# yhz0/SQLP

Hardware: AMD Instinct MI355X
Metric: stage-2 subproblems/sec + cut-gen HBM GB/s on STORM (higher is better)
Workload: dtype f64

## Files before the change

sqlp_amd/csrc/lp_batch.hip:

```cpp
#include <hip/hip_runtime.h>
#include <algorithm>
#include <cmath>
#include <cstdio>
#include <cstdlib>
#include <vector>
#include "twosd_internal.h"
#include "twosd_ctx.h"

using namespace twosd;

int twosd::run_lp(twosd_ctx *c, const double *x, const double *d_dv, int N, const LpRun &o) {
    const bool want_pi = o.want_pi, want_y = o.want_y;
    const bool list = o.d_list != nullptr;
    const int NL = list ? o.nlist : N;
    int rc;
    if (o.want_ray && !list) return fail(TWOSD_E_ARG, "LP rays: list mode only");
    if ((rc = prepare_x(c, x))) return rc;
    if (list &&c->bp.bases.size() > 1 && (size_t)N > c->d_pool_pick.cap) return fail(TWOSD_E_STATE, "LP list mode: no recorded pool picks");
    const int m = c->L.m, n = c->L.n, MP = c->MP, R = c->R;
    if (N > c->out_cap) {
        size_t cap = std::max<size_t>(N, 1024);
        if ((rc = c->d_obj.alloc(cap)) || (rc = c->d_status.alloc(cap)) || (rc = c->d_iters.alloc(cap)) ||
            (rc = c->d_ops.alloc(cap)) || (rc = c->d_etan.alloc(cap)))
            return rc;
// ... 17 lines not shown
        int bpc = hyper_max_blocks_per_cu(R, CH, kmax, c->k);
        if (const char *e = getenv("TWOSD_BPC")) bpc = std::min(bpc, std::max(1, atoi(e)));
        if (bpc < 1)
            return fail(TWOSD_E_UNSUPPORTED, "LP kernel: LDS slice too large (m2 = %d, n2 = %d; LP: %d rows, %d columns; k = %d)",
                        c->m2_user, c->n2_user, m, n, c->k);
        const int nblocks = std::max(1, std::min((NL + kWavesPerBlock - 1) / kWavesPerBlock, bpc * c->num_cus));
        const size_t slots = (size_t)nblocks * kWavesPerBlock;
        if (slots > c->earena_slots || ecap != c->earena_cap) {
            if ((rc = c->d_eidx.alloc(slots * ecap)) || (rc = c->d_evals.alloc(slots * ecap))) return rc;
            c->earena_slots = slots;
            c->earena_cap = ecap;
        }
        HIPCHK(hipMemsetAsync(c->d_queue, 0, sizeof(int) * kMaxQueueGroups * kQueueStride, c->stream));
        HyperParams H{};
        H.m = m; H.n = n; H.k = c->k; H.N = NL; H.kmax = kmax; H.ecap = ecap;
        H.kcap = o.kcap > 0 ? std::min(o.kcap, kmax) : kmax;
        H.retry = o.kcap > 0 ? 0 : 1;
        H.colptr = c->d_colptr; H.rowidx = c->d_rowidx; H.val = c->d_val; H.q = c->d_q; H.btype = c->d_btype;
        H.wcp = c->d_wcp; H.wcc = c->d_wcc; H.wcv = c->d_wcv;
        const PoolArrays pa = pool_arrays(c);
        H.bcp = pa.bcp; H.bci = pa.bci; H.bcv = pa.bcv;
        H.brptr = pa.brptr; H.brcol = pa.brcol; H.brval = pa.brval;
        H.kslot = pa.kslot; H.kix = pa.kix; H.kv = pa.kv; H.kcoef = c->d_kcoef;
        H.xbase = c->d_xbase; H.d0 = pa.d0; H.hb0 = pa.hb0;
        H.basic0 = pa.basic0; H.fixedmask = c->d_fixedmask; H.ubmask = c->d_ubmask;
        H.dv = d_dv; H.eidx = c->d_eidx; H.evals = c->d_evals; H.queue = c->d_queue;
        H.qgroups = std::max(1, std::min(16, nblocks));
        if (const char *e = getenv("TWOSD_QGROUPS")) H.qgroups = std::max(1, std::min({kMaxQueueGroups, nblocks, atoi(e)}));
        H.obj = c->d_obj; H.pi = want_pi ? c->d_pi : nullptr; H.y = want_y ? c->d_y : nullptr;
        H.vkey = o.want_key ? c->d_vkey : nullptr;
        H.key_zero = 1e-12;
        if (const char *e = getenv("TWOSD_KEY_ZERO")) H.key_zero = atof(e);
        H.bkey = o.want_bkey ? c->d_bkey : nullptr;
        if (o.want_etas) {
            const size_t need = list ? (size_t)NL : (size_t)N;
            if (need * 4096 > (size_t)INT32_MAX)
                return fail(TWOSD_E_UNSUPPORTED, "eta files of %zu solves exceed the 2^31-entry arena (at most %d)", need,
                            INT32_MAX / 4096);
            const size_t cap_need = std::max(std::max<size_t>(need, 256) * 4096, c->eo_min_cap);
            if (need > c->eo_rows || c->eo_kmax != kmax || c->eo_cap < cap_need) {
                const size_t rows = std::max<size_t>(need, 256);
                if ((rc = c->d_eo_pb.alloc(rows)) || (rc = c->d_eo_K.alloc(rows)) || (rc = c->d_eo_off.alloc(rows)) ||
                    (rc = c->d_eo_etap.alloc(rows * kmax)) || (rc = c->d_eo_etaoff.alloc(rows * (kmax + 1))) ||
                    (rc = c->d_eo_eidx.alloc(cap_need)) || (rc = c->d_eo_evals.alloc(cap_need)))
                    return rc;
                if (!c->d_eo_used && (rc = c->d_eo_used.alloc(1))) return rc;
                c->eo_rows = rows;
                c->eo_cap = cap_need;
                c->eo_kmax = kmax;
            }
            HIPCHK(hipMemsetAsync(c->d_eo_used, 0, sizeof(unsigned long long), c->stream));
            H.eo_pb = c->d_eo_pb; H.eo_K = c->d_eo_K; H.eo_off = c->d_eo_off; H.eo_etap = c->d_eo_etap;
            H.eo_etaoff = c->d_eo_etaoff; H.eo_eidx = c->d_eo_eidx; H.eo_evals = c->d_eo_evals; H.eo_used = c->d_eo_used;
            H.eo_cap = (long long)std::min<size_t>(c->eo_cap, INT32_MAX);
        }
        if (o.want_head) {
            const size_t need = list ? (size_t)NL : (size_t)N;
            if ((rc = c->d_head_out.fit(need * m))) return rc;
            H.head_out = c->d_head_out;
        }
        if (o.want_ray) {
            FrayState &Fs = c->fray;
            if ((rc = Fs.ray.fit((size_t)NL * m)) || (rc = Fs.ray_row.fit((size_t)NL)) || (rc = Fs.ray_key.fit((size_t)NL))) return rc;
            HIPCHK(hipMemsetAsync(Fs.ray_row, 0xff, sizeof(int) * NL, c->stream));
            HIPCHK(hipMemsetAsync(Fs.ray_key, 0, sizeof(unsigned long long) * NL, c->stream));
            H.ray = Fs.ray; H.ray_row = Fs.ray_row; H.ray_key = Fs.ray_key;
// ... 291 lines not shown
    if (row_ops) *row_ops = c->last.ops_sum;
    if (row_width) *row_width = 1;
    return TWOSD_OK;
}

__global__ void gather_rows_kernel(int U, int m, const int *__restrict__ list, const double *__restrict__ pi, double *__restrict__ out) {
    const size_t tot = (size_t)U * m;
    for (size_t i = (size_t)blockIdx.x * blockDim.x + threadIdx.x; i < tot; i += (size_t)gridDim.x * blockDim.x) {
        const int u = (int)(i / m), r = (int)(i % m);
        out[i] = pi[(size_t)list[u] * m + r];
    }
}

__global__ void list_status_kernel(int U, const int *__restrict__ list, const int *__restrict__ st,
                                   unsigned long long *bad) {
    for (int i = blockIdx.x * blockDim.x + threadIdx.x; i < U; i += gridDim.x * blockDim.x)
        if (st[list[i]] != TWOSD_LP_OPTIMAL) atomicAdd(bad, 1ull);
}

extern "C" int twosd_solve_push(twosd_ctx *c, int epi, const double *x, int first, int count, double *obj, int *status,
                                int *new_size) {
    if (!c || !c->has_template) return fail(TWOSD_E_STATE, "solve_push: no template");
    if (!c->bp.has_basis) return fail(TWOSD_E_STATE, "solve_push: no warm-start basis");
    if (epi < 0 || epi >= (int)c->epis.size()) return fail(TWOSD_E_ARG, "solve_push: epigraph %d does not exist", epi);
    const EpiDevice &E = c->epis[epi];
    if (first < 0 || count < 0 || first + count > E.count) return fail(TWOSD_E_ARG, "solve_push: range outside the epigraph");
    if (c->n1 > 0 && !x) return fail(TWOSD_E_ARG, "solve_push: x is NULL");
    if (count == 0) { if (new_size) *new_size = c->dvs.size; return TWOSD_OK; }
    HIPCHK(hipSetDevice(c->device));
    const double *d_dv = E.d_dv + (size_t)first * c->k;
    const bool all = getenv("TWOSD_PUSH_ALL") && atoi(getenv("TWOSD_PUSH_ALL")) != 0;
    const int pmode = getenv("TWOSD_PUSH_MODE") ? atoi(getenv("TWOSD_PUSH_MODE")) : 0;
    const bool full = !all && (pmode == 2 || (pmode == 0 && c->push_rep_frac > 0.25));
    c->last_push_full = full ? 1 : 0;
    LpRun o;
    o.want_pi = all || full;
    o.want_key = !all;
    int rc = run_lp(c, x, d_dv, count, o);
    if (rc) return rc;
    rc = copy_lp_outputs(c, count, obj, nullptr, nullptr, status, E.d_w + first);
    if (rc) return rc;
    float ms = 0, ms_key = 0;
    const auto timed_push = [c](int n, const double *d_rows, float *ms_out) -> int {
        HIPCHK(hipEventRecord(c->ev[EV_PUSH_BEGIN], c->stream));
        if (int r = dvs_push_device(c, n, d_rows, nullptr)) return r;
        HIPCHK(hipEventRecord(c->ev[EV_PUSH_END], c->stream));
        HIPCHK(hipEventSynchronize(c->ev[EV_PUSH_END]));
        hipEventElapsedTime(ms_out, c->ev[EV_PUSH_BEGIN], c->ev[EV_PUSH_END]);
        return TWOSD_OK;
    };
    if (all) {
        if ((rc = timed_push(count, c->d_pi, &ms))) return rc;
        c->last_push_reps = count;
    } else {
        HIPCHK(hipEventRecord(c->ev[EV_MARK_1], c->stream));
        const int *d_list = nullptr;
        int U = 0;
        if ((rc = vkey_first_occurrences(c, count, c->d_vkey, c->d_status, &d_list, &U))) return rc;
        HIPCHK(hipEventRecord(c->ev[EV_MARK_2], c->stream));
        HIPCHK(hipEventSynchronize(c->ev[EV_MARK_2]));
        hipEventElapsedTime(&ms_key, c->ev[EV_MARK_1], c->ev[EV_MARK_2]);
        c->last_push_reps = U;
        c->push_rep_frac = (double)U / count;
        if (U > 0 && full) {
            const int m = c->L.m;
            if ((rc = c->d_pi_rep.fit((size_t)U * m))) return rc;
            hipLaunchKernelGGL(gather_rows_kernel, dim3((unsigned)std::min<size_t>(4096, ((size_t)U * m + 255) / 256)), dim3(256), 0,
                               c->stream, U, m, d_list, c->d_pi, c->d_pi_rep);
            HIPCHK(hipGetLastError());
            if ((rc = timed_push(U, c->d_pi_rep, &ms))) return rc;
        } else if (U > 0) {
            double resolve_us = 0.0;
            LpRun r;
            r.want_pi = true;
            r.d_list = d_list;
            r.nlist = U;
            r.lp_us_out = &resolve_us;
            if ((rc = run_lp(c, x, d_dv, count, r))) return rc;
            HIPCHK(hipMemsetAsync(c->d_lpstats, 0, sizeof(unsigned long long), c->stream));
            hipLaunchKernelGGL(list_status_kernel, dim3((unsigned)std::min(256, (U + 255) / 256)), dim3(256), 0, c->stream, U,
                               d_list, c->d_status, c->d_lpstats);
            HIPCHK(hipGetLastError());
            unsigned long long bad = 0;
            HIPCHK(hipMemcpyAsync(&bad, c->d_lpstats, sizeof(bad), hipMemcpyDeviceToHost, c->stream));
            HIPCHK(hipStreamSynchronize(c->stream));
            if (bad) return fail(TWOSD_E_LP, "solve_push: %llu of %d re-solved representatives not optimal; nothing pushed", bad, U);
            c->last.lp_us += resolve_us;
            if ((rc = timed_push(U, c->d_pi, &ms))) return rc;
        }
    }
    c->t_us[T_DEDUP] = 1e3 * (ms + ms_key);
    if (new_size) *new_size = c->dvs.size;
    return TWOSD_OK;
}

extern "C" int twosd_last_push_mode(twosd_ctx *c, int *full) {
    if (!c || !full) return fail(TWOSD_E_ARG, "last_push_mode: NULL");
// ... 10 lines not shown
```

sqlp_amd/csrc/lp_hyper.hip:

```cpp
#include <hip/hip_runtime.h>
#include <math.h>
#include <type_traits>
#include "twosd_internal.h"
#include "wave_ops.h"

namespace twosd {

#define HTOL_P 1e-9
#define HTOL_D 1e-9
#define HTOL_PIV 1e-9
#define HPI_ZERO 1e-12


#ifdef TWOSD_STAMPS
#define STAMP_DECL unsigned long long st_acc[10] = {0, 0, 0, 0, 0, 0, 0, 0, 0, 0}; \
    unsigned long long st_last = __builtin_amdgcn_s_memtime();
#define STAMP(i)                                                      \
    {                                                                 \
        const unsigned long long t_ = __builtin_amdgcn_s_memtime();   \
        st_acc[i] += t_ - st_last;                                    \
        st_last = t_;                                                 \
    }
#define STAMP_FLUSH                                                                         \
    if (lane == 0 && P.stamps)                                                              \
// ... 116 lines not shown

__device__ __forceinline__ const __attribute__((address_space(4))) HyperParams *h_args() {
    uint64_t a = (uint64_t)__builtin_amdgcn_kernarg_segment_ptr();
    asm volatile("" : "+s"(a));
    return (const __attribute__((address_space(4))) HyperParams *)a;
}
#define CP (*h_args())

static __host__ __device__ inline int hyper_union_doubles(int R, int C) {
    return 128 * R > 64 * C ? 128 * R : 64 * C;
}
static __host__ __device__ inline size_t hyper_slice_bytes(int R, int C, int kmax, int k) {
    const int kmaxp = (kmax + 3) & ~3;
    return 8 * (size_t)hyper_union_doubles(R, C) + 8 * (size_t)((k + 1) & ~1) + 8 * 64 + 4 * 64 + 4 * 64 + 2 * kmaxp +
           4 * (kmaxp + 4);
}
size_t hyper_lds_bytes(int R, int C, int kmax, int k) { return (size_t)kWavesPerBlock * hyper_slice_bytes(R, C, kmax, k); }

#ifndef TWOSD_ETA_G
#define TWOSD_ETA_G 2
#endif
constexpr int EG = TWOSD_ETA_G;
#ifndef TWOSD_REC_UNROLL
#define TWOSD_REC_UNROLL 1
#endif
#ifndef TWOSD_XB_U
#define TWOSD_XB_U 1
#endif
constexpr int XU = TWOSD_XB_U;
#ifndef TWOSD_HYPER_WPE
#define TWOSD_HYPER_WPE(R) ((R) >= 9 ? 2 : 3)
#endif

template <int R, int C, bool FULL, bool RAY = false>
__global__ void __launch_bounds__(256, TWOSD_HYPER_WPE(R)) lp_hyper_kernel(HyperParams P) {
    extern __shared__ double lds_raw[];
    using Mask = typename std::conditional<(C > 32), uint64_t, uint32_t>::type;
    const int lane = threadIdx.x & 63;
    const int wid = threadIdx.x >> 6;
    constexpr int MP = 64 * R;
    constexpr int UD = 128 * R > 64 * C ? 128 * R : 64 * C;
    const int kmaxp = (P.kmax + 3) & ~3;
    const int ncol = P.n + P.m;
    char *slice = reinterpret_cast<char *>(lds_raw) + (size_t)wid * hyper_slice_bytes(R, C, P.kmax, P.k);
    double *ut = reinterpret_cast<double *>(slice);
    double *rho = ut + MP;
    double *alpha = ut;
    double *dvl = ut + UD;
    double *lstv = dvl + ((P.k + 1) & ~1);
    int *lsti = reinterpret_cast<int *>(lstv + 64);
    int *smark = lsti + 64;
    unsigned short *etap = reinterpret_cast<unsigned short *>(smark + 64);
    int *etaoff = reinterpret_cast<int *>(etap + kmaxp);

    const int m = P.m, n = P.n;
    const int slot_id = blockIdx.x * kWavesPerBlock + wid;
    int *eidx = P.eidx + (size_t)slot_id * P.ecap;
    double *evals = P.evals + (size_t)slot_id * P.ecap;
    const uint64_t fixedm = CP.fixedmask[lane];
    const uint64_t ubm = CP.ubmask[lane];

    for (int j = lane; j < UD; j += 64) ut[j] = 0.0;
    smark[lane] = 0;
    h_wave_sync();
    STAMP_DECL

    const int G = CP.qgroups;
    const int g0 = blockIdx.x % G;
// ... 539 lines not shown
                {
                    const int nh = q * 4 + (int)P.btype[q];
                    const bool rme = lane == (r & 63);
                    H_SLOT_SWITCH(__builtin_amdgcn_readfirstlane(r >> 6), R, {
                        int v = rme ? nh : hb[SL];
                        asm volatile("" : "+v"(v));
                        hb[SL] = v;
                    })
                }
            }
            ++it;
            h_wave_sync();
            STAMP(8)
        }
        if (status == TWOSD_LP_OPTIMAL || pb == 0 || !CP.retry) break;
        if (lane == 0 && CP.retries) atomicAdd(CP.retries, 1ull);
        pb = 0;
        }
        double dvn0 = 0.0, dvn1 = 0.0, kcn0 = 0.0, kcn1 = 0.0;
        int ksn = 0, t_claim = 0;
        if (q_nx >= 0) {
            const auto *A = h_args();
            t_claim = claim_issue();
            if (lane <= R) ksn = A->kslot[pb_nx * (R + 1) + lane];
            if (dv_pf) {
                const double *dvs = A->dv + (size_t)s_nx * P.k;
                if (lane < P.k) { dvn0 = dvs[lane]; kcn0 = A->kcoef[lane]; }
                if (lane + 64 < P.k) { dvn1 = dvs[lane + 64]; kcn1 = A->kcoef[lane + 64]; }
            }
        }

        double objv = NAN;
        unsigned long long keyv = 0;
        if (status == TWOSD_LP_OPTIMAL) {
            const double *qc = CP.q;
            double qv[R];
#pragma unroll
            for (int t = 0; t < R; ++t) {
                const int j = hb[t] >> 2;
                qv[t] = qc[(hb[t] >= 0 && j < n) ? j : 0];
            }
            double ob = 0.0;
#pragma unroll
            for (int t = 0; t < R; ++t) {
                const int j = hb[t] >> 2;
                ob = (hb[t] >= 0 && j < n) ? fma(qv[t], xB[t], ob) : ob;
            }
            objv = wsum(ob);
        }
        q_n2 = -1;
        if (q_nx >= 0) {
            q_n2 = claim_resolve(t_claim);
            if (lane <= R) lsti[lane] = ksn;
            if (dv_pf) {
                if (lane < P.k) dvl[lane] = kcn0 * dvn0;
                if (lane + 64 < P.k) dvl[lane + 64] = kcn1 * dvn1;
            }
        }
        h_wave_sync();
        if (status == TWOSD_LP_OPTIMAL) {
            if (CP.vkey) {
                uint64_t ub = ubm;
                int lane = threadIdx.x & 63;
                asm volatile("" : "+v"(ub), "+v"(lane));
                auto dk = [&](int c) -> double {
                    const int j = 64 * c + lane;
                    const bool slack = (j >= n) & (j < ncol) & (((bmask >> c) & 1) == 0);
                    return slack ? h_flip(d[c], ((ub >> c) & 1) << 63) : 0.0;
                };
                double pm = 0.0;
#pragma unroll
                for (int c = 0; c < C; ++c) pm = fmax(pm, fabs(dk(c)));
                pm = wmax(pm);
                const double zt = CP.key_zero * (1.0 + pm);
                unsigned long long h = 0;
#pragma unroll
                for (int c = 0; c < C; ++c) {
                    const int j = 64 * c + lane;
                    if (j >= n && j < ncol) {
                        const double dc = dk(c);
                        const double v = fabs(dc) <= zt ? 0.0 : dc;
                        const unsigned long long b = ((unsigned long long)__double_as_longlong(v) + (1ull << 28)) >> 29;
                        h += mix64(((unsigned long long)(j - n) << 35) | b);
                    }
                }
#pragma unroll
                for (int o = 32; o > 0; o >>= 1) h += __shfl_xor(h, o);
                keyv = h;
            }
        }
        if constexpr (FULL) {
        bool rayrec = false;
        if constexpr (RAY) rayrec = status == TWOSD_LP_INFEASIBLE && CP.ray != nullptr;
        if ((status == TWOSD_LP_OPTIMAL && (P.pi || P.y)) || rayrec) {
            if (rayrec) {
                if (lane == (ray_r & 63)) ut[ray_r] = 1.0;
            } else {
                const double *qc = CP.q;
#pragma unroll
                for (int t = 0; t < R; ++t) {
                    const int j = hb[t] >> 2;
                    const bool bq = hb[t] >= 0 && j < n;
                    const double qj = qc[bq ? j : 0];
                    ut[64 * t + lane] = bq ? qj : 0.0;
                }
            }
            h_wave_sync();
            for (int tt = K - 1; tt >= 0; --tt) {
                const int off = etaoff[tt], nnz = etaoff[tt + 1] - off;
                double acc = 0.0;
                for (int e = lane; e < nnz; e += 64) acc = fma(ut[eidx[off + e]], evals[off + e], acc);
                acc = wsum(acc);
                nops += nnz;
                if (lane == 0) ut[etap[tt]] = acc;
                h_wave_sync();
            }
            double pv[R];
            double pmax = 0.0;
#pragma unroll
            for (int t = 0; t < R; ++t) {
                const int cc = 64 * t + lane;
                const int e0 = cc < m ? bcp[cc] : 0, e1 = cc < m ? bcp[cc + 1] : 0;
                double a = 0.0;
#pragma unroll TWOSD_REC_UNROLL
                for (int e = e0; e < e1; ++e) a = fma(ut[P.bci[e]], P.bcv[e], a);
                pv[t] = a;
                pmax = fmax(pmax, fabs(a));
            }
            nops += P.bnnz[pb];
            pmax = wmax(pmax);
            const double zt = HPI_ZERO * (1.0 + pmax);
#pragma unroll
            for (int t = 0; t < R; ++t)
                if (fabs(pv[t]) <= zt) pv[t] = 0.0;
            h_wave_sync();
#pragma unroll
            for (int t = 0; t < R; ++t) ut[64 * t + lane] = 0.0;
            if constexpr (RAY) {
                if (rayrec) {
                    const auto *A = h_args();
                    const size_t ro = (size_t)(P.pi_by_pos ? qpos : s);
                    double *po = A->ray + ro * m;
                    const uint64_t sm = ray_up ? 0ull : (1ull << 63);
                    unsigned long long h = 0;
#pragma unroll
                    for (int t = 0; t < R; ++t)
                        if (64 * t + lane < m) {
                            po[64 * t + lane] = pv[t] == 0.0 ? 0.0 : h_flip(pv[t], sm);
                            h += mix64((unsigned long long)(hb[t] >> 2));
                        }
#pragma unroll
                    for (int o = 32; o > 0; o >>= 1) h += __shfl_xor(h, o);
                    const int leaving = h_get_row_i<R>(hb, ray_r) >> 2;
                    if (lane == 0) {
                        if (A->ray_row) A->ray_row[ro] = ray_r;
                        if (A->ray_key) A->ray_key[ro] = mix64(h ^ mix64(((unsigned long long)leaving << 1) | (ray_up ? 1ull : 0ull)));
                    }
                }
            }
            if (!rayrec && P.pi) {
                double *po = P.pi + (size_t)(P.pi_by_pos ? qpos : s) * m;
#pragma unroll
                for (int t = 0; t < R; ++t)
                    if (64 * t + lane < m) po[64 * t + lane] = pv[t];
            }
            if (!rayrec && P.y) {
                double *yo = P.y + (size_t)s * n;
                for (int j = lane; j < n; j += 64) yo[j] = 0.0;
                __builtin_amdgcn_s_waitcnt(0);
                __builtin_amdgcn_wave_barrier();
// ... 332 lines not shown
__global__ void __launch_bounds__(256) queue_records_kernel(int N, const int *__restrict__ order, const int *__restrict__ pick,
                                                           int2 *__restrict__ qrec) {
    const int q = blockIdx.x * blockDim.x + threadIdx.x;
    if (q >= N) return;
    const int s = order ? order[q] : q;
    qrec[q] = make_int2(s, pick ? pick[s] : 0);
}
hipError_t launch_queue_records(const int *order, const int *pick, int2 *qrec, int N, hipStream_t s) {
    if (N <= 0) return hipSuccess;
    hipLaunchKernelGGL(queue_records_kernel, dim3((N + 255) / 256), dim3(256), 0, s, N, order, pick, qrec);
    return hipGetLastError();
}

static const int kHR[] = {1, 2, 4, 9, 16};
static const int kHC[] = {2, 4, 8, 14, 16, 28, 32, 64};

int hyper_rows_per_lane(int m) {
    for (int R : kHR)
        if (m <= 64 * R) return R;
    return -1;
}
int hyper_cols_per_lane(int ncols) {
    for (int C : kHC)
        if (ncols <= 64 * C) return C;
    return -1;
}

template <int R, int C>
static hipError_t hl(const HyperParams &p, int nb, size_t lds, hipStream_t s) {
    if (p.ray)
        hipLaunchKernelGGL((lp_hyper_kernel<R, C, true, true>), dim3(nb), dim3(256), lds, s, p);
    else if (p.pi || p.y || p.head_out || p.bkey || p.eo_K)
        hipLaunchKernelGGL((lp_hyper_kernel<R, C, true>), dim3(nb), dim3(256), lds, s, p);
    else
        hipLaunchKernelGGL((lp_hyper_kernel<R, C, false>), dim3(nb), dim3(256), lds, s, p);
    return hipGetLastError();
}
template <int R, int C>
static int ho(size_t lds) {
    int nb = 0, nb2 = 0;
    if (hipOccupancyMaxActiveBlocksPerMultiprocessor(&nb, lp_hyper_kernel<R, C, true>, 256, lds) != hipSuccess) return 1;
    if (hipOccupancyMaxActiveBlocksPerMultiprocessor(&nb2, lp_hyper_kernel<R, C, false>, 256, lds) != hipSuccess) return 1;
    nb = std::min(nb, nb2);
    return nb > 0 ? nb : 1;
}

#ifdef HYP_DEV_STORM_ONLY
#define HYPER_C_SWITCH(R, FN, ...)                  \
    switch (C) {                                    \
        case 28: if (R == 9) return FN<9, 28>(__VA_ARGS__); \
    }
#else
#define HYPER_C_SWITCH(R, FN, ...)                  \
    switch (C) {                                    \
        case 2: return FN<R, 2>(__VA_ARGS__);       \
        case 4: return FN<R, 4>(__VA_ARGS__);       \
        case 8: return FN<R, 8>(__VA_ARGS__);       \
        case 14: return FN<R, 14>(__VA_ARGS__);     \
        case 16: return FN<R, 16>(__VA_ARGS__);     \
        case 28: return FN<R, 28>(__VA_ARGS__);     \
        case 32: return FN<R, 32>(__VA_ARGS__);     \
        case 64: return FN<R, 64>(__VA_ARGS__);     \
    }
#endif

hipError_t launch_hyper(int R, int C, const HyperParams &p, int nblocks, size_t lds, hipStream_t s) {
    switch (R) {
        case 1: HYPER_C_SWITCH(1, hl, p, nblocks, lds, s); break;
        case 2: HYPER_C_SWITCH(2, hl, p, nblocks, lds, s); break;
        case 4: HYPER_C_SWITCH(4, hl, p, nblocks, lds, s); break;
        case 9: HYPER_C_SWITCH(9, hl, p, nblocks, lds, s); break;
        case 16: HYPER_C_SWITCH(16, hl, p, nblocks, lds, s); break;
    }
    return hipErrorInvalidValue;
}

// ... 15 lines not shown
```

sqlp_amd/csrc/twosd_ctx.h:

```cpp
#pragma once
#include <hip/hip_runtime.h>
#include <stdint.h>
#include <algorithm>
#include <memory>
#include <thread>
#include <vector>
#include "devbuf.h"
#include "twosd_internal.h"
#include "basis_pool.h"

#define HIPCHK(expr)                                                                                      \
    do {                                                                                                  \
        hipError_t _e = (expr);                                                                           \
        if (_e != hipSuccess) return twosd::fail(TWOSD_E_DEVICE, "%s: %s", #expr, hipGetErrorString(_e)); \
    } while (0)

namespace twosd {

enum StageSlot : int {
    STG_POOL_RCOL = 0, STG_POOL_CROW, STG_POOL_RVAL, STG_POOL_CVAL, STG_POOL_D0,
    STG_ELEM_KE, STG_ELEM_KIX, STG_ELEM_KRAW, STG_ELEM_KV,
    STG_PG_TOT,
    STG_FREE_10,
    STG_PG_NZ,
// ... 236 lines not shown
    twosd::DevBuf<char> d_rt_pack;
    twosd::DevBuf<int> d_gs_heads, d_gs_cnt, d_gs_tot, d_gs_valid, d_gs_irow;
    twosd::DevBuf<long long> d_gs_ioff;
    twosd::DevBuf<double> d_gs_ival;
    twosd::DevBuf<char> d_gs_seg;
    int last_push_reps = 0;
    double push_rep_frac = 0.0;
    int last_push_full = 0;
    twosd::DevBuf<double> d_pi_rep;
    twosd::FrayState fray;
    twosd::RiskState risk;
};

struct twosd_ctx : TemplateState {
    int device = 0;
    hipStream_t stream = nullptr;
    hipEvent_t ev[twosd::EV_COUNT] = {};
    int num_cus = 256;
    int kmax_override = 0;
    int train_kcap = 0;
    twosd::PinnedBuf stage[twosd::STG_COUNT];
    ~twosd_ctx() {
        for (hipEvent_t e : ev)
            if (e) hipEventDestroy(e);
        if (stream) hipStreamDestroy(stream);
    }
};

namespace twosd {
int fail(int code, const char *fmt, ...);
int prepare_x(twosd_ctx *c, const double *x);
struct LpRun {
    bool want_pi = false, want_y = false, want_key = false;
    bool want_bkey = false;
    bool want_etas = false;
    bool want_head = false;
    const int *d_list = nullptr;
    int nlist = 0;
    int kcap = 0;
    double *lp_us_out = nullptr;
    bool want_ray = false;
};
int run_lp(twosd_ctx *c, const double *x, const double *d_dv, int N, const LpRun &o = LpRun());
#pragma GCC visibility push(hidden)
double template_value(const twosd_ctx *c, int e);
void rhs_at(const twosd_ctx *c, const double *x, const double *dv, std::vector<double> &b);
SampleParams sample_params(const twosd_ctx *c, int n, uint64_t seed, uint64_t first_index, double *out);
int draw_scenarios(twosd_ctx *c, int n, uint64_t seed, uint64_t first_index, double *out, int mode, int G);
int upload_lintr(twosd_ctx *c, const LintrTables &T);
int select_pool(twosd_ctx *c, const double *d_dv, int N, int *d_pick, int npool_override);
int copy_lp_outputs(twosd_ctx *c, int N, double *obj, double *pi, double *y, int *status, const double *d_w);
int prepare_elements(twosd_ctx *c);
int reserve_selection(twosd_ctx *c, int P, int records);
void reset_candidates(twosd_ctx *c);
int training_box(twosd_ctx *c, const EpiDevice &E, int epi, int first, int count, std::vector<double> &lo,
                 std::vector<double> &hi, BoxCache *cache);
#pragma GCC visibility pop
template <typename F>
void parallel_for(int n, F f, int serial_below = 64) {
    const int nth = (int)std::max(1u, std::min(16u, std::thread::hardware_concurrency()));
    if (n < serial_below || nth == 1) {
        for (int i = 0; i < n; ++i) f(i);
        return;
    }
    std::vector<std::thread> th;
    for (int t = 0; t < nth; ++t)
        th.emplace_back([&, t]() {
            for (int i = t; i < n; i += nth) f(i);
        });
    for (auto &t : th) t.join();
}
int vkey_first_occurrences(twosd_ctx *c, int N, const unsigned long long *d_vkey, const int *d_status, const int **d_list,
                           int *U, const int **d_counts = nullptr);
int dvs_init(twosd_ctx *c);
int dvs_push_device(twosd_ctx *c, int count, const double *d_pis, int *d_out_index);
void cut_invalidate_pk(twosd_ctx *c);
void cut_truncate_pk(twosd_ctx *c, int size);
int cut_last_usable(twosd_ctx *c, int epi, const char *who, const char *verb);
const int *cut_last_arg(twosd_ctx *c);
int cut_pk_current(twosd_ctx *c, const double **PK, int *k4);
const double *cut_last_val(twosd_ctx *c);
struct RiskResult { double var, cvar; unsigned long long tail_q, total_q; long long n_bad, n_ok; };
int risk_select(twosd_ctx *c, long long n, const double *d_val, const double *d_w, const int *d_st, double scale, bool has_add,
                double add, double level, const char *who, RiskResult *out);
int risk_form_y(twosd_ctx *c, long long n, double *d_obj, const int *d_st, double var, double denom);
int sampling_plan(const twosd_sampling *plan, const char *who, int *mode, int *G);
int whole_groups(const char *who, const char *what, unsigned long long value, int G);
}
```

sqlp_amd/csrc/twosd_internal.h:

```cpp
#pragma once
#include <hip/hip_runtime.h>
#include <stdint.h>
#include <string>
#include <vector>
#include "twosd_hip.h"
#include "devbuf.h"
#include "dist_tables.h"
#include "lintr_tables.h"
#include "pool_pack.h"

namespace twosd {

constexpr int kWave = 64;
constexpr int kWavesPerBlock = 4;
constexpr int kMaxColsPerLane = 64;

enum : int { BT_Y = 0, BT_G = 1, BT_L = 2, BT_E = 3 };


constexpr int kQueueStride = 32;
constexpr int kMaxQueueGroups = 64;
struct HyperParams {
    int m, n, k, N, kmax, ecap;
    int kcap;
    int retry;
    const int *colptr, *rowidx; const double *val;
    const double *q; const int8_t *btype;
    const int *wcp, *wcc; const double *wcv;
    const int *bcp, *bci; const double *bcv;
    const int *brptr, *brcol; const double *brval;
    const int *kslot, *kix; const double *kv;
    const double *kcoef;
    const double *xbase;
    const double *d0;
    const int *hb0;
    const uint64_t *basic0, *fixedmask, *ubmask;
    const double *dv;
    int *eidx; double *evals;
    int *queue;
    int qgroups;
    double *obj;
    int *status, *iters;
    long long *ops;
    int *etan;
    int *pool_pick;
    unsigned long long *vkey;
    double *pi, *y;
    unsigned long long *retries;
    unsigned long long *stamps;
    int npool;
    const int *bnnz;
    int *head_out;
    const int2 *qrec;
    double key_zero;
    int pi_by_pos;
    unsigned long long *bkey;
    int *eo_pb, *eo_K, *eo_off, *eo_etap, *eo_etaoff;
    int *eo_eidx; double *eo_evals;
    unsigned long long *eo_used; long long eo_cap;
    double *ray;
    int *ray_row;
    unsigned long long *ray_key;
};

struct PgArgs {
    int m, n, MP, CH, R9, k, kmax, npool_old;
    const int *colptr, *rowidx; const double *val, *q; const int8_t *btype; const int *pos_row;
    const int *bcp0, *bci0; const double *bcv0;
    const int *eo_pb, *eo_K, *eo_off, *eo_etap, *eo_etaoff, *eo_eidx; const double *eo_evals;
    const int *head0, *heads;
    const int *src_row;
    const int *gheads;
    int a0;
    double *amax;
    int *nzc, *keptc;
    int *nztot;
    const long long *inter_off;
    int *inter_row; double *inter_val;
    int *rowcnt, *erowcnt;
    int *tot;
    int *valid;
    long long sc_cap;
    int *sc_row, *sc_off; double *sc_val;
};
struct PgTable {
    int nsrc;
    int *cnt, *tot, *valid;
    long long *ioff;
    int *irow;
    double *ival;
    int *gheads;
    static size_t plane_size(int nsrc, int m) { return (size_t)nsrc * m; }
    static size_t cnt_size(int nsrc, int m) { return 4 * plane_size(nsrc, m); }
    static size_t tot_size(int nsrc) { return (size_t)5 * nsrc; }
    int *plane(int f, int m) const { return cnt + f * plane_size(nsrc, m); }
// ... 123 lines not shown
```

sqlp_amd/csrc/vkey.hip:

```cpp
#include <hip/hip_runtime.h>
#include <hipcub/hipcub.hpp>
#include <algorithm>
#include "twosd_ctx.h"

namespace twosd {

__device__ __forceinline__ unsigned long long vk_norm(unsigned long long k) { return k ? k : 1ull; }
__device__ __forceinline__ unsigned vk_slot(unsigned long long k, unsigned mask) {
    return (unsigned)((k * 0x9E3779B97F4A7C15ull) >> 32) & mask;
}

__global__ void vkey_clear_kernel(unsigned long long *keys, int *first, int *cnt, unsigned cap) {
    for (unsigned i = blockIdx.x * blockDim.x + threadIdx.x; i < cap; i += gridDim.x * blockDim.x) {
        keys[i] = 0ull;
        first[i] = 0x7fffffff;
        cnt[i] = 0;
    }
}

constexpr int kVkItems = 2048;
constexpr int kVkLds = 2 * kVkItems;
__global__ void __launch_bounds__(256) vkey_insert_kernel(int N, const unsigned long long *__restrict__ vkey,
                                                          const int *__restrict__ status, unsigned long long *keys,
                                                          int *first, int *cnt, unsigned mask) {
    __shared__ unsigned long long lk[kVkLds];
    __shared__ int lf[kVkLds], lc[kVkLds];
    for (int i = threadIdx.x; i < kVkLds; i += blockDim.x) {
        lk[i] = 0ull;
        lf[i] = 0x7fffffff;
        lc[i] = 0;
    }
    __syncthreads();
    const int s0 = blockIdx.x * kVkItems, s1 = min(N, s0 + kVkItems);
    for (int s = s0 + threadIdx.x; s < s1; s += blockDim.x) {
        if (status[s] != TWOSD_LP_OPTIMAL) continue;
        const unsigned long long k = vk_norm(vkey[s]);
        unsigned i = vk_slot(k, kVkLds - 1);
        for (;;) {
            const unsigned long long old = atomicCAS(&lk[i], 0ull, k);
            if (old == 0ull || old == k) {
                atomicMin(&lf[i], s);
                atomicAdd(&lc[i], 1);
                break;
// ... 23 lines not shown
                                  int *out) {
    for (int a = blockIdx.x * blockDim.x + threadIdx.x; a < U; a += gridDim.x * blockDim.x) {
        const unsigned long long k = vk_norm(vkey[list[a]]);
        unsigned i = vk_slot(k, mask);
        while (keys[i] != k) i = (i + 1) & mask;
        out[a] = cnt[i];
    }
}

__global__ void vkey_flag_kernel(int N, const unsigned long long *__restrict__ vkey, const int *__restrict__ status,
                                 const unsigned long long *__restrict__ keys, const int *__restrict__ first,
                                 unsigned mask, char *flag) {
    for (int s = blockIdx.x * blockDim.x + threadIdx.x; s < N; s += gridDim.x * blockDim.x) {
        char f = 0;
        if (status[s] == TWOSD_LP_OPTIMAL) {
            const unsigned long long k = vk_norm(vkey[s]);
            unsigned i = vk_slot(k, mask);
            while (keys[i] != k) i = (i + 1) & mask;
            f = first[i] == s;
        }
        flag[s] = f;
    }
}

template <typename T>
using WsBuf = DevBuf<T, 8>;
struct VkeyWs {
    WsBuf<unsigned long long> keys;
    WsBuf<int> first, cnt;
    unsigned cap = 0;
    WsBuf<char> flag;
    WsBuf<int> list, counts, nsel;
    WsBuf<char> tmp;
};

static VkeyWs *vws(twosd_ctx *c) {
    if (!c->vkey_ws) c->vkey_ws.reset(new VkeyWs());
    return c->vkey_ws.get();
}

void vkey_free(VkeyWs *w) { delete w; }

int vkey_first_occurrences(twosd_ctx *c, int N, const unsigned long long *d_vkey, const int *d_status, const int **d_list,
                           int *U, const int **d_counts) {
    VkeyWs *w = vws(c);
    unsigned cap = 1024;
    while (cap < 2u * (unsigned)N) cap <<= 1;
    int rc;
    if (cap > w->cap) {
        w->cap = 0;
        if ((rc = w->keys.alloc(cap)) || (rc = w->first.alloc(cap)) || (rc = w->cnt.alloc(cap))) return rc;
        w->cap = cap;
    }
    if ((rc = w->flag.fit((size_t)N)) || (rc = w->list.fit((size_t)N)) || (rc = w->counts.fit((size_t)N))) return rc;
    if (!w->nsel && (rc = w->nsel.alloc(1))) return rc;
    size_t need = 0;
    HIPCHK(hipcub::DeviceSelect::Flagged(nullptr, need, hipcub::CountingInputIterator<int>(0), w->flag.p, w->list.p, w->nsel.p, N,
                                         c->stream));
    if ((rc = w->tmp.fit(need))) return rc;
    const unsigned mask = w->cap - 1;
    const int nb = std::max(1, std::min(4096, (N + 255) / 256));
    hipLaunchKernelGGL(vkey_clear_kernel, dim3(std::min(4096u, (w->cap + 255) / 256)), dim3(256), 0, c->stream, w->keys, w->first,
                       w->cnt, w->cap);
    hipLaunchKernelGGL(vkey_insert_kernel, dim3(std::max(1, (N + kVkItems - 1) / kVkItems)), dim3(256), 0, c->stream, N, d_vkey, d_status,
                       w->keys, w->first, w->cnt, mask);
    hipLaunchKernelGGL(vkey_flag_kernel, dim3(nb), dim3(256), 0, c->stream, N, d_vkey, d_status, w->keys, w->first, mask,
                       w->flag);
    HIPCHK(hipGetLastError());
    HIPCHK(hipcub::DeviceSelect::Flagged(w->tmp.p, need, hipcub::CountingInputIterator<int>(0), w->flag.p, w->list.p, w->nsel.p, N,
                                         c->stream));
    HIPCHK(hipMemcpyAsync(U, w->nsel, sizeof(int), hipMemcpyDeviceToHost, c->stream));
    HIPCHK(hipStreamSynchronize(c->stream));
    *d_list = w->list;
    if (d_counts) {
        if (*U > 0) {
            hipLaunchKernelGGL(vkey_count_kernel, dim3(std::max(1, std::min(4096, (*U + 255) / 256))), dim3(256), 0, c->stream, *U,
                               w->list, d_vkey, w->keys, w->cnt, mask, w->counts);
            HIPCHK(hipGetLastError());
        }
        *d_counts = w->counts;
    }
    return TWOSD_OK;
}

}
```

Before: 18.26 million.

## Dedupe dual keys inside the LP kernel and recover duals only for representatives

Adds a REP variant of the lean hyper-sparse LP kernel. Each solve computes its dual key, claims a slot in a global hash table with atomics, and only the lowest-index owner of each key recovers and writes its dual vector, so push no longer needs a separate full dual-recovery pass or host-side dedupe kernels in the common mode. A small winner/gather pass then selects the final representatives, with a fallback to the old vkey path if the table overflows or counts disagree. The cost is extra atomics and global traffic inside the kernel, some wasted recoveries when a lower-index owner arrives later, and a third kernel variant that may lower the occupancy chosen for all variants.

```diff
diff --git a/sqlp_amd/csrc/lp_batch.hip b/sqlp_amd/csrc/lp_batch.hip
--- a/sqlp_amd/csrc/lp_batch.hip
+++ b/sqlp_amd/csrc/lp_batch.hip
@@ -73,6 +73,7 @@
         H.key_zero = 1e-12;
         if (const char *e = getenv("TWOSD_KEY_ZERO")) H.key_zero = atof(e);
         H.bkey = o.want_bkey ? c->d_bkey : nullptr;
+        if (o.want_rep && o.want_key && !list && !want_pi && !want_y && (rc = rep_prepare(c, N, H))) return rc;
         if (o.want_etas) {
             const size_t need = list ? (size_t)NL : (size_t)N;
             if (need * 4096 > (size_t)INT32_MAX)
@@ -430,10 +431,12 @@
     const bool all = getenv("TWOSD_PUSH_ALL") && atoi(getenv("TWOSD_PUSH_ALL")) != 0;
     const int pmode = getenv("TWOSD_PUSH_MODE") ? atoi(getenv("TWOSD_PUSH_MODE")) : 0;
     const bool full = !all && (pmode == 2 || (pmode == 0 && c->push_rep_frac > 0.25));
+    const bool inpass = !all && !full && (pmode == 3 || pmode == 0);
     c->last_push_full = full ? 1 : 0;
     LpRun o;
     o.want_pi = all || full;
     o.want_key = !all;
+    o.want_rep = inpass;
     int rc = run_lp(c, x, d_dv, count, o);
     if (rc) return rc;
     rc = copy_lp_outputs(c, count, obj, nullptr, nullptr, status, E.d_w + first);
@@ -454,13 +457,20 @@
         HIPCHK(hipEventRecord(c->ev[EV_MARK_1], c->stream));
         const int *d_list = nullptr;
         int U = 0;
-        if ((rc = vkey_first_occurrences(c, count, c->d_vkey, c->d_status, &d_list, &U))) return rc;
+        bool got = false;
+        if (inpass && (rc = rep_winners(c, count, c->d_vkey, &U, &got))) return rc;
+        if (!got) {
+            if ((rc = vkey_first_occurrences(c, count, c->d_vkey, c->d_status, &d_list, &U))) return rc;
+            if (inpass) rep_note_reps(c, U);
+        }
         HIPCHK(hipEventRecord(c->ev[EV_MARK_2], c->stream));
         HIPCHK(hipEventSynchronize(c->ev[EV_MARK_2]));
         hipEventElapsedTime(&ms_key, c->ev[EV_MARK_1], c->ev[EV_MARK_2]);
         c->last_push_reps = U;
         c->push_rep_frac = (double)U / count;
-        if (U > 0 && full) {
+        if (U > 0 && got) {
+            if ((rc = timed_push(U, c->d_pi_rep, &ms))) return rc;
+        } else if (U > 0 && full) {
             const int m = c->L.m;
             if ((rc = c->d_pi_rep.fit((size_t)U * m))) return rc;
             hipLaunchKernelGGL(gather_rows_kernel, dim3((unsigned)std::min<size_t>(4096, ((size_t)U * m + 255) / 256)), dim3(256), 0,
diff --git a/sqlp_amd/csrc/lp_hyper.hip b/sqlp_amd/csrc/lp_hyper.hip
--- a/sqlp_amd/csrc/lp_hyper.hip
+++ b/sqlp_amd/csrc/lp_hyper.hip
@@ -172,8 +172,97 @@
 #define TWOSD_HYPER_WPE(R) ((R) >= 9 ? 2 : 3)
 #endif
 
-template <int R, int C, bool FULL, bool RAY = false>
+template <int R>
+__device__ __forceinline__ void h_recover(double (&pv)[R], const HyperParams &P, bool rayrec, int ray_r, const int (&hb)[R], int K,
+                                          int pb, double *ut, const int *etaoff, const unsigned short *etap, const int *eidx,
+                                          const double *evals, const int *bcp, unsigned &nops, int lane) {
+    const int m = P.m, n = P.n;
+    if (rayrec) {
+        if (lane == (ray_r & 63)) ut[ray_r] = 1.0;
+    } else {
+        const double *qc = CP.q;
+#pragma unroll
+        for (int t = 0; t < R; ++t) {
+            const int j = hb[t] >> 2;
+            const bool bq = hb[t] >= 0 && j < n;
+            const double qj = qc[bq ? j : 0];
+            ut[64 * t + lane] = bq ? qj : 0.0;
+        }
+    }
+    h_wave_sync();
+    for (int tt = K - 1; tt >= 0; --tt) {
+        const int off = etaoff[tt], nnz = etaoff[tt + 1] - off;
+        double acc = 0.0;
+        for (int e = lane; e < nnz; e += 64) acc = fma(ut[eidx[off + e]], evals[off + e], acc);
+        acc = wsum(acc);
+        nops += nnz;
+        if (lane == 0) ut[etap[tt]] = acc;
+        h_wave_sync();
+    }
+    double pmax = 0.0;
+#pragma unroll
+    for (int t = 0; t < R; ++t) {
+        const int cc = 64 * t + lane;
+        const int e0 = cc < m ? bcp[cc] : 0, e1 = cc < m ? bcp[cc + 1] : 0;
+        double a = 0.0;
+#pragma unroll TWOSD_REC_UNROLL
+        for (int e = e0; e < e1; ++e) a = fma(ut[P.bci[e]], P.bcv[e], a);
+        pv[t] = a;
+        pmax = fmax(pmax, fabs(a));
+    }
+    nops += P.bnnz[pb];
+    pmax = wmax(pmax);
+    const double zt = HPI_ZERO * (1.0 + pmax);
+#pragma unroll
+    for (int t = 0; t < R; ++t)
+        if (fabs(pv[t]) <= zt) pv[t] = 0.0;
+    h_wave_sync();
+#pragma unroll
+    for (int t = 0; t < R; ++t) ut[64 * t + lane] = 0.0;
+}
+
+typedef unsigned rep_u4 __attribute__((ext_vector_type(4)));
+__device__ __forceinline__ rep_u4 rep_probe(RepEntry *e) {
+#ifdef TWOSD_REP_PROBE_SC1
+    const unsigned long long k = __hip_atomic_load(&e->key, __ATOMIC_RELAXED, __HIP_MEMORY_SCOPE_AGENT);
+    const int o = __hip_atomic_load(&e->owner, __ATOMIC_RELAXED, __HIP_MEMORY_SCOPE_AGENT);
+    return (rep_u4){(unsigned)k, (unsigned)(k >> 32), (unsigned)o, 0u};
+#else
+    return *reinterpret_cast<const rep_u4 *>(e);
+#endif
+}
+
+#define H_DUAL_KEY(keyv)                                                                                         \
+    {                                                                                                            \
+        uint64_t ub = ubm;                                                                                       \
+        int lane = threadIdx.x & 63;                                                                             \
+        asm volatile("" : "+v"(ub), "+v"(lane));                                                                 \
+        auto dk = [&](int c) -> double {                                                                         \
+            const int j = 64 * c + lane;                                                                         \
+            const bool slack = (j >= n) & (j < ncol) & (((bmask >> c) & 1) == 0);                                \
+            return slack ? h_flip(d[c], ((ub >> c) & 1) << 63) : 0.0;                                            \
+        };                                                                                                       \
+        double pm = 0.0;                                                                                         \
+        _Pragma("unroll") for (int c = 0; c < C; ++c) pm = fmax(pm, fabs(dk(c)));                                \
+        pm = wmax(pm);                                                                                           \
+        const double zt = CP.key_zero * (1.0 + pm);                                                              \
+        unsigned long long h = 0;                                                                                \
+        _Pragma("unroll") for (int c = 0; c < C; ++c) {                                                          \
+            const int j = 64 * c + lane;                                                                         \
+            if (j >= n && j < ncol) {                                                                            \
+                const double dc = dk(c);                                                                         \
+                const double v = fabs(dc) <= zt ? 0.0 : dc;                                                      \
+                const unsigned long long b = ((unsigned long long)__double_as_longlong(v) + (1ull << 28)) >> 29; \
+                h += mix64(((unsigned long long)(j - n) << 35) | b);                                             \
+            }                                                                                                    \
+        }                                                                                                        \
+        _Pragma("unroll") for (int o = 32; o > 0; o >>= 1) h += __shfl_xor(h, o);                                \
+        keyv = h;                                                                                                \
+    }
+
+template <int R, int C, bool FULL, bool RAY = false, bool REP = false>
 __global__ void __launch_bounds__(256, TWOSD_HYPER_WPE(R)) lp_hyper_kernel(HyperParams P) {
+    static_assert(!(REP && FULL), "REP is a variant of the lean kernel");
     extern __shared__ double lds_raw[];
     using Mask = typename std::conditional<(C > 32), uint64_t, uint32_t>::type;
     const int lane = threadIdx.x & 63;
@@ -779,6 +868,22 @@
 
         double objv = NAN;
         unsigned long long keyv = 0;
+        unsigned long long rkey = 0;
+        unsigned rhome = 0;
+        rep_u4 rprobe = {0u, 0u, (unsigned)kRepNoOwner, 0u};
+        int rflags = 0;
+        if constexpr (REP) {
+            if (status == TWOSD_LP_OPTIMAL) {
+                const auto *A = h_args();
+                H_DUAL_KEY(keyv)
+                rkey = vk_norm(keyv);
+                rhome = vk_slot(rkey, A->rep_mask);
+                int hv = (int)rhome, fv = REP_FLAGS;
+                asm volatile("" : "+v"(hv), "+v"(fv));
+                rprobe = rep_probe(A->rep_tab + hv);
+                rflags = A->rep_ctl[fv];
+            }
+        }
         if (status == TWOSD_LP_OPTIMAL) {
             const double *qc = CP.q;
             double qv[R];
@@ -805,84 +910,62 @@
             }
         }
         h_wave_sync();
+        if constexpr (!REP) {
         if (status == TWOSD_LP_OPTIMAL) {
             if (CP.vkey) {
-                uint64_t ub = ubm;
-                int lane = threadIdx.x & 63;
-                asm volatile("" : "+v"(ub), "+v"(lane));
-                auto dk = [&](int c) -> double {
-                    const int j = 64 * c + lane;
-                    const bool slack = (j >= n) & (j < ncol) & (((bmask >> c) & 1) == 0);
-                    return slack ? h_flip(d[c], ((ub >> c) & 1) << 63) : 0.0;
-                };
-                double pm = 0.0;
-#pragma unroll
-                for (int c = 0; c < C; ++c) pm = fmax(pm, fabs(dk(c)));
-                pm = wmax(pm);
-                const double zt = CP.key_zero * (1.0 + pm);
-                unsigned long long h = 0;
-#pragma unroll
-                for (int c = 0; c < C; ++c) {
-                    const int j = 64 * c + lane;
-                    if (j >= n && j < ncol) {
-                        const double dc = dk(c);
-                        const double v = fabs(dc) <= zt ? 0.0 : dc;
-                        const unsigned long long b = ((unsigned long long)__double_as_longlong(v) + (1ull << 28)) >> 29;
-                        h += mix64(((unsigned long long)(j - n) << 35) | b);
+                H_DUAL_KEY(keyv)
+            }
+        }
+        } else if (status == TWOSD_LP_OPTIMAL) {
+            const unsigned long long pk = ((unsigned long long)rprobe.y << 32) | rprobe.x;
+            const bool settled = ((pk == rkey) & ((int)rprobe.z <= s)) | (rflags != 0);
+            if (!__builtin_amdgcn_readfirstlane((int)settled)) {
+                const auto *A = h_args();
+                int slot = -1;
+                if (lane == 0) {
+                    RepEntry *tab = A->rep_tab;
+                    int *ctl = A->rep_ctl;
+                    const unsigned mask = A->rep_mask;
+                    unsigned i = rhome;
+                    bool found = false;
+                    for (int t = 0; t < kRepProbes; ++t) {
+                        const unsigned long long old = atomicCAS(&tab[i].key, 0ull, rkey);
+                        if (old == 0ull || old == rkey) {
+                            if (old == 0ull) atomicAdd(&ctl[REP_KEYS], 1);
+                            found = true;
+                            break;
+                        }
+                        i = (i + 1) & mask;
                     }
-                }
-#pragma unroll
-                for (int o = 32; o > 0; o >>= 1) h += __shfl_xor(h, o);
-                keyv = h;
+                    if (!found) {
+                        atomicOr(&ctl[REP_FLAGS], 1);
+                    } else if (atomicMin(&tab[i].owner, s) > s) {
+                        slot = atomicAdd(&ctl[REP_COUNT], 1);
+                        if (slot >= A->rep_rows) {
+                            atomicOr(&ctl[REP_FLAGS], 2);
+                            slot = -1;
+                        }
+                    }
+                }
+                slot = __builtin_amdgcn_readfirstlane(slot);
+                if (slot >= 0) {
+                    double pv[R];
+                    unsigned rops = 0;
+                    h_recover<R>(pv, P, false, 0, hb, K, pb, ut, etaoff, etap, eidx, evals, bcp, rops, lane);
+                    double *po = A->rep_pi + (size_t)slot * m;
+#pragma unroll
+                    for (int t = 0; t < R; ++t)
+                        if (64 * t + lane < m) po[64 * t + lane] = pv[t];
+                    if (lane == 0) A->rep_scen[slot] = s;
+                }
             }
         }
         if constexpr (FULL) {
         bool rayrec = false;
         if constexpr (RAY) rayrec = status == TWOSD_LP_INFEASIBLE && CP.ray != nullptr;
         if ((status == TWOSD_LP_OPTIMAL && (P.pi || P.y)) || rayrec) {
-            if (rayrec) {
-                if (lane == (ray_r & 63)) ut[ray_r] = 1.0;
-            } else {
-                const double *qc = CP.q;
-#pragma unroll
-                for (int t = 0; t < R; ++t) {
-                    const int j = hb[t] >> 2;
-                    const bool bq = hb[t] >= 0 && j < n;
-                    const double qj = qc[bq ? j : 0];
-                    ut[64 * t + lane] = bq ? qj : 0.0;
-                }
-            }
-            h_wave_sync();
-            for (int tt = K - 1; tt >= 0; --tt) {
-                const int off = etaoff[tt], nnz = etaoff[tt + 1] - off;
-                double acc = 0.0;
-                for (int e = lane; e < nnz; e += 64) acc = fma(ut[eidx[off + e]], evals[off + e], acc);
-                acc = wsum(acc);
-                nops += nnz;
-                if (lane == 0) ut[etap[tt]] = acc;
-                h_wave_sync();
-            }
             double pv[R];
-            double pmax = 0.0;
-#pragma unroll
-            for (int t = 0; t < R; ++t) {
-                const int cc = 64 * t + lane;
-                const int e0 = cc < m ? bcp[cc] : 0, e1 = cc < m ? bcp[cc + 1] : 0;
-                double a = 0.0;
-#pragma unroll TWOSD_REC_UNROLL
-                for (int e = e0; e < e1; ++e) a = fma(ut[P.bci[e]], P.bcv[e], a);
-                pv[t] = a;
-                pmax = fmax(pmax, fabs(a));
-            }
-            nops += P.bnnz[pb];
-            pmax = wmax(pmax);
-            const double zt = HPI_ZERO * (1.0 + pmax);
-#pragma unroll
-            for (int t = 0; t < R; ++t)
-                if (fabs(pv[t]) <= zt) pv[t] = 0.0;
-            h_wave_sync();
-#pragma unroll
-            for (int t = 0; t < R; ++t) ut[64 * t + lane] = 0.0;
+            h_recover<R>(pv, P, rayrec, ray_r, hb, K, pb, ut, etaoff, etap, eidx, evals, bcp, nops, lane);
             if constexpr (RAY) {
                 if (rayrec) {
                     const auto *A = h_args();
@@ -1281,16 +1364,19 @@
         hipLaunchKernelGGL((lp_hyper_kernel<R, C, true, true>), dim3(nb), dim3(256), lds, s, p);
     else if (p.pi || p.y || p.head_out || p.bkey || p.eo_K)
         hipLaunchKernelGGL((lp_hyper_kernel<R, C, true>), dim3(nb), dim3(256), lds, s, p);
+    else if (p.rep_tab)
+        hipLaunchKernelGGL((lp_hyper_kernel<R, C, false, false, true>), dim3(nb), dim3(256), lds, s, p);
     else
         hipLaunchKernelGGL((lp_hyper_kernel<R, C, false>), dim3(nb), dim3(256), lds, s, p);
     return hipGetLastError();
 }
 template <int R, int C>
 static int ho(size_t lds) {
-    int nb = 0, nb2 = 0;
+    int nb = 0, nb2 = 0, nb3 = 0;
     if (hipOccupancyMaxActiveBlocksPerMultiprocessor(&nb, lp_hyper_kernel<R, C, true>, 256, lds) != hipSuccess) return 1;
     if (hipOccupancyMaxActiveBlocksPerMultiprocessor(&nb2, lp_hyper_kernel<R, C, false>, 256, lds) != hipSuccess) return 1;
-    nb = std::min(nb, nb2);
+    if (hipOccupancyMaxActiveBlocksPerMultiprocessor(&nb3, lp_hyper_kernel<R, C, false, false, true>, 256, lds) != hipSuccess) return 1;
+    nb = std::min({nb, nb2, nb3});
     return nb > 0 ? nb : 1;
 }
 
diff --git a/sqlp_amd/csrc/twosd_ctx.h b/sqlp_amd/csrc/twosd_ctx.h
--- a/sqlp_amd/csrc/twosd_ctx.h
+++ b/sqlp_amd/csrc/twosd_ctx.h
@@ -292,6 +292,7 @@
 int prepare_x(twosd_ctx *c, const double *x);
 struct LpRun {
     bool want_pi = false, want_y = false, want_key = false;
+    bool want_rep = false;
     bool want_bkey = false;
     bool want_etas = false;
     bool want_head = false;
@@ -332,6 +333,9 @@
 }
 int vkey_first_occurrences(twosd_ctx *c, int N, const unsigned long long *d_vkey, const int *d_status, const int **d_list,
                            int *U, const int **d_counts = nullptr);
+int rep_prepare(twosd_ctx *c, int N, HyperParams &H);
+int rep_winners(twosd_ctx *c, int N, const unsigned long long *d_vkey, int *U, bool *ok);
+void rep_note_reps(twosd_ctx *c, int U);
 int dvs_init(twosd_ctx *c);
 int dvs_push_device(twosd_ctx *c, int count, const double *d_pis, int *d_out_index);
 void cut_invalidate_pk(twosd_ctx *c);
diff --git a/sqlp_amd/csrc/twosd_internal.h b/sqlp_amd/csrc/twosd_internal.h
--- a/sqlp_amd/csrc/twosd_internal.h
+++ b/sqlp_amd/csrc/twosd_internal.h
@@ -20,6 +20,18 @@
 
 constexpr int kQueueStride = 32;
 constexpr int kMaxQueueGroups = 64;
+__host__ __device__ inline unsigned long long vk_norm(unsigned long long k) { return k ? k : 1ull; }
+__host__ __device__ inline unsigned vk_slot(unsigned long long k, unsigned mask) {
+    return (unsigned)((k * 0x9E3779B97F4A7C15ull) >> 32) & mask;
+}
+struct alignas(16) RepEntry {
+    unsigned long long key;
+    int owner;
+    int pad;
+};
+constexpr int kRepNoOwner = 0x7fffffff;
+constexpr int kRepProbes = 64;
+enum : int { REP_COUNT = 0, REP_FLAGS = 1, REP_KEYS = 2, REP_CTL_WORDS = 4 };
 struct HyperParams {
     int m, n, k, N, kmax, ecap;
     int kcap;
@@ -61,6 +73,12 @@
     double *ray;
     int *ray_row;
     unsigned long long *ray_key;
+    RepEntry *rep_tab;
+    unsigned rep_mask;
+    int rep_rows;
+    double *rep_pi;
+    int *rep_scen;
+    int *rep_ctl;
 };
 
 struct PgArgs {
diff --git a/sqlp_amd/csrc/vkey.hip b/sqlp_amd/csrc/vkey.hip
--- a/sqlp_amd/csrc/vkey.hip
+++ b/sqlp_amd/csrc/vkey.hip
@@ -4,11 +4,6 @@
 #include "twosd_ctx.h"
 
 namespace twosd {
-
-__device__ __forceinline__ unsigned long long vk_norm(unsigned long long k) { return k ? k : 1ull; }
-__device__ __forceinline__ unsigned vk_slot(unsigned long long k, unsigned mask) {
-    return (unsigned)((k * 0x9E3779B97F4A7C15ull) >> 32) & mask;
-}
 
 __global__ void vkey_clear_kernel(unsigned long long *keys, int *first, int *cnt, unsigned cap) {
     for (unsigned i = blockIdx.x * blockDim.x + threadIdx.x; i < cap; i += gridDim.x * blockDim.x) {
@@ -98,6 +93,13 @@
     WsBuf<char> flag;
     WsBuf<int> list, counts, nsel;
     WsBuf<char> tmp;
+    WsBuf<RepEntry> rep_tab;
+    WsBuf<double> rep_pi;
+    WsBuf<int> rep_scen, rep_ctl, rep_rowof;
+    unsigned rep_cap = 1u << 17;
+    unsigned rep_used = 0;
+    int rep_rows = 0;
+    int rep_last_u = 0;
 };
 
 static VkeyWs *vws(twosd_ctx *c) {
@@ -149,4 +151,95 @@
     return TWOSD_OK;
 }
 
-}
+
+__global__ void rep_clear_kernel(RepEntry *tab, unsigned cap, int *ctl) {
+    const unsigned t0 = blockIdx.x * blockDim.x + threadIdx.x;
+    for (unsigned i = t0; i < cap; i += gridDim.x * blockDim.x) tab[i] = RepEntry{0ull, kRepNoOwner, 0};
+    if (t0 < (unsigned)REP_CTL_WORDS) ctl[t0] = 0;
+}
+
+__global__ void rep_winner_kernel(int rows, const int *__restrict__ scen, const unsigned long long *__restrict__ vkey,
+                                  const RepEntry *__restrict__ tab, unsigned mask, const int *__restrict__ ctl, char *flag, int *rowof) {
+    const int count = min(ctl[REP_COUNT], rows);
+    for (int j = blockIdx.x * blockDim.x + threadIdx.x; j < count; j += gridDim.x * blockDim.x) {
+        const int s = scen[j];
+        const unsigned long long k = vk_norm(vkey[s]);
+        unsigned i = vk_slot(k, mask);
+        for (int t = 0; t < kRepProbes && tab[i].key != k; ++t) i = (i + 1) & mask;
+        if (tab[i].key == k && tab[i].owner == s) {
+            flag[s] = 1;
+            rowof[s] = j;
+        }
+    }
+}
+
+__global__ void rep_gather_kernel(int U, int m, const int *__restrict__ list, const int *__restrict__ rowof,
+                                  const double *__restrict__ pi, double *__restrict__ out) {
+    const size_t tot = (size_t)U * m;
+    for (size_t i = (size_t)blockIdx.x * blockDim.x + threadIdx.x; i < tot; i += (size_t)gridDim.x * blockDim.x) {
+        const int u = (int)(i / m), r = (int)(i % m);
+        out[i] = pi[(size_t)rowof[list[u]] * m + r];
+    }
+}
+
+int rep_prepare(twosd_ctx *c, int N, HyperParams &H) {
+    VkeyWs *w = vws(c);
+    const int m = c->L.m;
+    unsigned used = 1024;
+    while (used < 2u * (unsigned)N && used < w->rep_cap) used <<= 1;
+    int rows = std::min(std::max(4096, 4 * w->rep_last_u), std::max(N, 1));
+    if (const char *e = getenv("TWOSD_REP_TABLE"))
+        while (used > 1u && used > (unsigned)std::max(1, atoi(e))) used >>= 1;
+    if (const char *e = getenv("TWOSD_REP_ROWS")) rows = std::max(1, std::min(rows, atoi(e)));
+    int rc;
+    if ((rc = w->rep_tab.fit(used)) || (rc = w->rep_pi.fit((size_t)rows * m)) || (rc = w->rep_scen.fit((size_t)rows))) return rc;
+    if (!w->rep_ctl && (rc = w->rep_ctl.alloc(REP_CTL_WORDS))) return rc;
+    hipLaunchKernelGGL(rep_clear_kernel, dim3(std::max(1u, std::min(1024u, (used + 255) / 256))), dim3(256), 0, c->stream, w->rep_tab.p,
+                       used, w->rep_ctl.p);
+    HIPCHK(hipGetLastError());
+    w->rep_used = used;
+    w->rep_rows = rows;
+    H.rep_tab = w->rep_tab; H.rep_mask = used - 1; H.rep_rows = rows;
+    H.rep_pi = w->rep_pi; H.rep_scen = w->rep_scen; H.rep_ctl = w->rep_ctl;
+    return TWOSD_OK;
+}
+
+int rep_winners(twosd_ctx *c, int N, const unsigned long long *d_vkey, int *U, bool *ok) {
+    VkeyWs *w = vws(c);
+    const int m = c->L.m;
+    *U = 0;
+    *ok = false;
+    int rc;
+    if ((rc = w->flag.fit((size_t)N)) || (rc = w->list.fit((size_t)N)) || (rc = w->rep_rowof.fit((size_t)N))) return rc;
+    if (!w->nsel && (rc = w->nsel.alloc(1))) return rc;
+    size_t need = 0;
+    HIPCHK(hipcub::DeviceSelect::Flagged(nullptr, need, hipcub::CountingInputIterator<int>(0), w->flag.p, w->list.p, w->nsel.p, N,
+                                         c->stream));
+    if ((rc = w->tmp.fit(need))) return rc;
+    HIPCHK(hipMemsetAsync(w->flag, 0, (size_t)N, c->stream));
+    hipLaunchKernelGGL(rep_winner_kernel, dim3(std::max(1, std::min(1024, (w->rep_rows + 255) / 256))), dim3(256), 0, c->stream,
+                       w->rep_rows, w->rep_scen.p, d_vkey, w->rep_tab.p, w->rep_used - 1, w->rep_ctl.p, w->flag.p, w->rep_rowof.p);
+    HIPCHK(hipGetLastError());
+    HIPCHK(hipcub::DeviceSelect::Flagged(w->tmp.p, need, hipcub::CountingInputIterator<int>(0), w->flag.p, w->list.p, w->nsel.p, N,
+                                         c->stream));
+    int ctl[REP_CTL_WORDS], n = 0;
+    HIPCHK(hipMemcpyAsync(ctl, w->rep_ctl, sizeof(ctl), hipMemcpyDeviceToHost, c->stream));
+    HIPCHK(hipMemcpyAsync(&n, w->nsel, sizeof(int), hipMemcpyDeviceToHost, c->stream));
+    HIPCHK(hipStreamSynchronize(c->stream));
+    if ((ctl[REP_FLAGS] & 1) && w->rep_cap < (1u << 28)) w->rep_cap <<= 1;
+    if (ctl[REP_FLAGS] != 0 || n != ctl[REP_KEYS] || n < 0 || n > N) return TWOSD_OK;
+    if (n > 0) {
+        if ((rc = c->d_pi_rep.fit((size_t)n * m))) return rc;
+        hipLaunchKernelGGL(rep_gather_kernel, dim3((unsigned)std::min<size_t>(4096, ((size_t)n * m + 255) / 256)), dim3(256), 0, c->stream, n,
+                           m, w->list.p, w->rep_rowof.p, w->rep_pi.p, c->d_pi_rep.p);
+        HIPCHK(hipGetLastError());
+    }
+    w->rep_last_u = n;
+    *U = n;
+    *ok = true;
+    return TWOSD_OK;
+}
+
+void rep_note_reps(twosd_ctx *c, int U) { vws(c)->rep_last_u = U; }
+
+}
```

Result: slower. 17.99 million (-1.5%).
